# sid2364/dna-sequences-pg-extension

Measured on AMD Instinct MI355X. Metric: k-mers/sec for k=31 count over 3 Gbase synthetic; % of HBM-read roofline, higher is better.
Workload: dtype u64; 1 GPU; config 4: k=31 count over 3000000000 synthetic bases (splitmix64 seed 0xd2a0003), unordered groups (super-k-mer partitioning), single GPU; n_bases=3000000000, k=31, distinct=2999999968

## Files before the change

dna-sequences-pg-extension_amd/csrc/dnagpu_api.hip:

```cpp
#include "host_common.hpp"

using namespace dnagpu;

static thread_local char g_err[512] = "";

void dnagpu::set_err(const char *fmt, ...)
{
    va_list ap;
    va_start(ap, fmt);
    vsnprintf(g_err, sizeof g_err, fmt, ap);
    va_end(ap);
}

extern "C" const char *dnagpu_strerror(int status)
{
    switch (status) {
    case DNAGPU_OK: return "ok";
    case DNAGPU_ERR_INVALID_K: return "Invalid k value: must be between 1 and 32";
    case DNAGPU_ERR_QKMER_LEN_MISMATCH: return "Qkmer pattern and kmer lengths do not match";
    case DNAGPU_ERR_PREFIX_TOO_LONG: return "Prefix length cannot exceed kmer length";
    case DNAGPU_ERR_QKMER_INVALID: return "Invalid Qkmer sequence: must contain valid IUPAC nucleotide codes";
    case DNAGPU_ERR_BAD_ARG: return "bad argument";
    case DNAGPU_ERR_TOO_LARGE: return "too many k-mers for one call (limit 2^32 - 1)";
    case DNAGPU_ERR_NO_DEVICE: return "no usable HIP device (gfx950 required)";
// ... 133 lines not shown
#endif
    if (e != hipSuccess) {
        (void)hipGetLastError();
        hipStreamSynchronize(ctx->stream);
        for (size_t i = 0; i < ctx->pool.size();) {
            if (!ctx->pool[i].in_use) {
                hipFree(ctx->pool[i].ptr);
                ctx->pool.erase(ctx->pool.begin() + i);
            } else {
                i++;
            }
        }
        e = hipMalloc(&p, want);
    }
    if (e != hipSuccess) {
        (void)hipGetLastError();
        set_err("hipMalloc(%zu bytes) failed: %s", want, hipGetErrorString(e));
        return DNAGPU_ERR_OOM;
    }
    ctx->pool.push_back(PoolBlock{p, want, true});
    return finish(ctx->pool.back());
}

static int pool_check_guards(dnagpu_ctx *ctx)
{
    if (!(ctx->debug_flags & DNAGPU_DEBUG_GUARD_POOL))
        return DNAGPU_OK;
    unsigned char band[POOL_GUARD];
    for (const PoolBlock &b : ctx->pool) {
        if (!b.guard_at)
            continue;
        HIP_TRY(hipMemcpy(band, static_cast<const char *>(b.ptr) + b.guard_at, POOL_GUARD, hipMemcpyDeviceToHost));
        for (size_t i = 0; i < POOL_GUARD; i++)
            if (band[i] != 0xA5) {
                set_err("pool guard: a kernel wrote %zu bytes past the end of a %zu-byte work buffer (%s)", i + 1, b.guard_at,
                        b.in_use ? "in use" : "already returned");
                return DNAGPU_ERR_INTERNAL;
            }
    }
    return DNAGPU_OK;
}

void dnagpu::pool_free(dnagpu_ctx *ctx, void *p)
{
    if (!p)
        return;
    for (PoolBlock &b : ctx->pool)
        if (b.ptr == p) {
            b.in_use = false;
            return;
        }
}

HistPtr dnagpu::hist_new(u64 total, bool sorted)
{
    HistPtr h(new (std::nothrow) dnagpu_hist());
    if (h) {
        h->total = total;
        h->sorted = sorted;
    }
    return h;
}

void dnagpu::hist_adopt(PoolScope &ps, dnagpu_hist *h, u64 *keys, u32 *counts, u64 *seg_off, u32 *seg_cnt, u32 n_segs, u64 n_distinct,
                        bool sorted, u64 extent)
{
    h->keys = keys;
    h->counts = counts;
    h->seg_off = seg_off;
    h->seg_cnt = seg_cnt;
    h->n_segs = n_segs;
    h->n_distinct = n_distinct;
    h->sorted = sorted;
    h->extent = extent;
    ps.release(keys);
    ps.release(counts);
    ps.release(seg_off);
    ps.release(seg_cnt);
}

int dnagpu::hist_adopt_one_segment(dnagpu_ctx *ctx, PoolScope &ps, dnagpu_hist *h, u64 *keys, u32 *counts, u64 n_groups, bool sorted)
{
    u64 *dir = nullptr;
    RC_TRY(ps.alloc(2, &dir));
    const u32 words[3] = {0, 0, (u32)n_groups};
    HIP_TRY(poke(dir, words, sizeof words, ctx->stream));
    HIP_TRY(hipStreamSynchronize(ctx->stream));
    hist_adopt(ps, h, keys, counts, dir, reinterpret_cast<u32 *>(dir + 1), 1, n_groups, sorted, 0);
    return DNAGPU_OK;
}

extern "C" int dnagpu_init(int device, dnagpu_ctx **out_ctx)
{
    return guarded([&]() -> int {
    if (!out_ctx)
        return DNAGPU_ERR_BAD_ARG;
    *out_ctx = nullptr;
    int n = 0;
    hipError_t e = hipGetDeviceCount(&n);
    if (e != hipSuccess || n <= 0) {
        (void)hipGetLastError();
        set_err("hipGetDeviceCount: %s (%d devices)", hipGetErrorString(e), n);
        return DNAGPU_ERR_NO_DEVICE;
    }
    if (device < 0 || device >= n) {
        set_err("device %d out of range (%d devices)", device, n);
        return DNAGPU_ERR_NO_DEVICE;
    }
    HIP_TRY(hipSetDevice(device));
    dnagpu_ctx *ctx = new (std::nothrow) dnagpu_ctx();
    if (!ctx)
        return DNAGPU_ERR_OOM;
    ctx->device = device;
    ctx->profiling = false;
    ctx->last_times.n = 0;
    e = hipStreamCreateWithFlags(&ctx->stream, hipStreamNonBlocking);
    if (e != hipSuccess) {
        set_err("hipStreamCreate: %s", hipGetErrorString(e));
        delete ctx;
        return DNAGPU_ERR_HIP;
    }
    ctx->mailbox = nullptr;
    ctx->debug_flags = 0;
    e = hipHostMalloc(reinterpret_cast<void **>(&ctx->mailbox), MAILBOX_BYTES, hipHostMallocDefault);
    if (e == hipSuccess)
        memset(ctx->mailbox, 0, MAILBOX_BYTES);
    if (e != hipSuccess) {
        set_err("hipHostMalloc: %s", hipGetErrorString(e));
        hipStreamDestroy(ctx->stream);
        delete ctx;
        return DNAGPU_ERR_OOM;
    }
    *out_ctx = ctx;
    return DNAGPU_OK;
    });
}

extern "C" void dnagpu_destroy(dnagpu_ctx *ctx)
{
    if (!ctx)
        return;
    hipSetDevice(ctx->device);
    hipStreamSynchronize(ctx->stream);
    for (PoolBlock &b : ctx->pool)
        hipFree(b.ptr);
    for (hipEvent_t e : ctx->ev)
        hipEventDestroy(e);
    hipStreamDestroy(ctx->stream);
    if (ctx->mailbox)
        hipHostFree(ctx->mailbox);
    delete ctx;
}

extern "C" int dnagpu_synchronize(dnagpu_ctx *ctx)
{
    return guarded([&]() -> int {
    if (!ctx)
        return DNAGPU_ERR_BAD_ARG;
    HIP_TRY(hipStreamSynchronize(ctx->stream));
    return pool_check_guards(ctx);
    });
}

extern "C" void *dnagpu_stream(dnagpu_ctx *ctx) { return ctx ? (void *)ctx->stream : nullptr; }

extern "C" int dnagpu_trim(dnagpu_ctx *ctx)
{
    return guarded([&]() -> int {
    if (!ctx)
        return DNAGPU_ERR_BAD_ARG;
    HIP_TRY(hipStreamSynchronize(ctx->stream));
    for (size_t i = 0; i < ctx->pool.size();) {
        if (!ctx->pool[i].in_use) {
            hipFree(ctx->pool[i].ptr);
            ctx->pool.erase(ctx->pool.begin() + i);
        } else {
            i++;
        }
    }
    return DNAGPU_OK;
    });
}

extern "C" uint64_t dnagpu_device_bytes(dnagpu_ctx *ctx)
{
    uint64_t t = 0;
    if (ctx)
        for (PoolBlock &b : ctx->pool)
            t += b.size;
    return t;
}

extern "C" int dnagpu_buffer_alloc(dnagpu_ctx *ctx, uint64_t bytes, void **dev_ptr)
{
    return guarded([&]() -> int {
    if (!ctx || !dev_ptr)
        return DNAGPU_ERR_BAD_ARG;
    HIP_TRY(hipSetDevice(ctx->device));
    return pool_alloc(ctx, (size_t)bytes, dev_ptr);
    });
// ... 1075 lines not shown
```

dna-sequences-pg-extension_amd/csrc/host_common.hpp:

```cpp
#pragma once
#include <hip/hip_runtime.h>

#include <algorithm>
#include <atomic>
#include <chrono>
#include <cmath>
#include <cstdarg>
#include <cstdio>
#include <cstdlib>
#include <cstring>
#include <initializer_list>
#include <memory>
#include <new>
#include <vector>

#include "../../include/dnagpu.h"
#include "kernels.hpp"

namespace dnagpu {
void set_err(const char *fmt, ...);

#ifdef DNAGPU_STAMPS
inline const char *diag_env(const char *name) { return getenv(name); }
#else
// ... 5 lines not shown
        hipError_t e_ = (expr);                                                              \
        if (e_ != hipSuccess) {                                                              \
            set_err("%s failed: %s (%s:%d)", #expr, hipGetErrorString(e_), __FILE__, __LINE__); \
            return e_ == hipErrorOutOfMemory ? DNAGPU_ERR_OOM : DNAGPU_ERR_HIP;              \
        }                                                                                    \
    } while (0)

#define RC_TRY(expr)           \
    do {                       \
        int rc_ = (expr);      \
        if (rc_ != DNAGPU_OK)  \
            return rc_;        \
    } while (0)

template <typename F>
int guarded(F &&body) noexcept
{
    try {
        return body();
    } catch (const std::bad_alloc &) {
        set_err("host allocation failed");
        return DNAGPU_ERR_OOM;
    } catch (...) {
        set_err("unexpected C++ exception");
        return DNAGPU_ERR_INTERNAL;
    }
}

struct PoolBlock {
    void *ptr;
    size_t size;
    bool in_use;
    size_t guard_at = 0;
};
constexpr size_t POOL_GUARD = 256;

constexpr size_t MAILBOX_BYTES = (size_t)1 << 20;

}
using dnagpu::u32;
using dnagpu::u64;

struct dnagpu_ctx {
    int device;
    hipStream_t stream;
    std::vector<dnagpu::PoolBlock> pool;
    bool profiling;
    dnagpu_phase_times last_times;
    std::vector<hipEvent_t> ev;
    std::vector<const char *> ev_names;
    u64 *mailbox;
    u64 mailbox_seq = 0;
    unsigned debug_flags;
};

struct dnagpu_dna {
    u64 *words;
    u64 n_words;
    u64 n_bases;
    bool owned;
    u64 *seq_starts = nullptr;
    u32 *seq_marks = nullptr;
    u64 n_seqs = 0, n_mark_words = 0;
};

struct dnagpu_hist {
    u64 *keys = nullptr;
    u32 *counts = nullptr;
    u64 n_distinct = 0;
    u64 total = 0;
    u64 *seg_off = nullptr;
    u32 *seg_cnt = nullptr;
    u32 *seg_pre = nullptr;
    u32 n_segs = 0;
    bool sorted = true;
    u64 extent = 0;
    std::vector<dnagpu_hist *> parts;
    int k = 0;
};
using HistPtr = std::unique_ptr<dnagpu_hist>;

namespace dnagpu {
hipError_t poke(void *dst, const void *src, size_t bytes, hipStream_t st);
int read_back(dnagpu_ctx *ctx, void *host, const void *dev, size_t bytes);

int pool_alloc(dnagpu_ctx *ctx, size_t bytes, void **out);
void pool_free(dnagpu_ctx *ctx, void *p);

template <typename T>
int pool_alloc_t(dnagpu_ctx *ctx, size_t n, T **out)
{
    void *p = nullptr;
    int rc = pool_alloc(ctx, n * sizeof(T), &p);
    *out = static_cast<T *>(p);
    return rc;
}

struct PoolScope {
    dnagpu_ctx *ctx;
    std::vector<void *> ptrs;
    explicit PoolScope(dnagpu_ctx *c) : ctx(c) {}
    ~PoolScope()
    {
        for (void *p : ptrs)
            pool_free(ctx, p);
    }
    template <typename T>
    int alloc(size_t n, T **out)
    {
        int rc = pool_alloc_t(ctx, n, out);
        if (rc == DNAGPU_OK)
            ptrs.push_back(*out);
        return rc;
    }
    void release(void *p)
    {
        ptrs.erase(std::remove(ptrs.begin(), ptrs.end(), p), ptrs.end());
    }
    void free_now(void *p)
    {
        release(p);
        pool_free(ctx, p);
    }
};

HistPtr hist_new(u64 total, bool sorted = true);
void hist_adopt(PoolScope &ps, dnagpu_hist *h, u64 *keys, u32 *counts, u64 *seg_off, u32 *seg_cnt, u32 n_segs, u64 n_distinct,
                bool sorted, u64 extent);
int hist_adopt_one_segment(dnagpu_ctx *ctx, PoolScope &ps, dnagpu_hist *h, u64 *keys, u32 *counts, u64 n_groups, bool sorted);

void prof_begin(dnagpu_ctx *ctx);
void prof_mark(dnagpu_ctx *ctx, const char *name);
void prof_end(dnagpu_ctx *ctx);

inline u64 words_for(u64 n_bases) { return (n_bases + 31) / 32; }
int check_range(const dnagpu_dna *dna, int k, u64 first, u64 count);

#pragma GCC visibility push(hidden)
constexpr u64 U32_MAX64 = 0xFFFFFFFFull;

// ... 151 lines not shown
```

dna-sequences-pg-extension_amd/csrc/sk_host.hip:

```cpp
#include "host_common.hpp"

using namespace dnagpu;


constexpr u64 SK_LEAF_MEAN = 2500;
constexpr u64 SK_MID_LIMIT = (u64)1 << 27;
#ifndef SK_MID_RECORDS_LOG2
#define SK_MID_RECORDS_LOG2 16
#endif
constexpr u32 SK_MID_RECORDS = 1u << SK_MID_RECORDS_LOG2;
constexpr u64 SK_BIG_LIMIT = 0xFFFFFFFFull;
constexpr int SK_B1_MAX = 9;
constexpr u64 SK_SLAB_MIN_ROWS = (u64)1 << 29;

template <typename T>
static int alloc1(PoolScope &ps, size_t n, T **out, size_t per = 1)
{
    return ps.alloc(std::max<size_t>(n, 1) * per, out);
}

static u32 sk_chunk_len(u64 x, u64 target = 4096, u64 tile = 8192)
{
    const u64 len = std::max<u64>(4 * tile, (x + target - 1) / target);
    return (u32)((len + tile - 1) / tile * tile);
// ... 122 lines not shown
static int sk_level0(dnagpu_ctx *ctx, PoolScope &ps, SkParts &p, const SkRows &rows, bool room_for_level1)
{
    hipStream_t st = ctx->stream;
    const dnagpu_dna *dna = rows.dna;
    const int k = p.k, b1 = p.g.b1, r0bits = p.g.r0bits;
    const u32 c0n = p.g.c0n;
    Node *cur = nullptr;
    u32 chunk_rows = 0;
    SkLevel l0;
    RC_TRY(sk_level0_begin(ctx, ps, rows.n, r0bits, 4096, &cur, &chunk_rows, &l0));
    prof_mark(ctx, "sk_hist0");
    HIP_TRY(launch_sk_level0(false, l0.chunks, l0.n_chunks, dna->words, dna->n_words, rows.first, k, c0n, (u32)b1, (u32)r0bits,
                             l0.hist, nullptr, nullptr, st, nullptr, rows.marks, rows.n_mark_words));
    prof_mark(ctx, "sk_prefix0");
    HIP_TRY(launch_level_prefix(cur, l0.chunks, l0.n_chunks, 1, chunk_rows, l0.hist, l0.tot, st));
    HIP_TRY(launch_level_children(cur, 1, l0.tot, l0.next, nullptr, nullptr, nullptr, 0, st));
    std::vector<Node> kids(l0.n_next);
    RC_TRY(read_back(ctx, kids.data(), l0.next, (size_t)l0.n_next * sizeof(Node)));
    std::vector<u32> &lens = p.lens;
    lens.resize(kids.size());
    u64 n_recs = 0;
    for (size_t i = 0; i < kids.size(); i++) {
        lens[i] = kids[i].len;
        n_recs += kids[i].len;
    }
    if (n_recs > 0xFFFFFFFFull)
        return DNAGPU_ERR_TOO_LARGE;
    void *rec0 = nullptr;
    u64 cap = std::max<u64>(n_recs, 1);
    if (room_for_level1) {
        u64 span = 0;
        const bool even = sk_even(lens.data(), (u32)lens.size(), 1.02, b1, &span);
        if (span <= 0xFFFFFFFFull)
            cap = std::max(cap, span);
        if ((ctx->debug_flags & DNAGPU_DEBUG_SAMPLE1) || !even) {
            const u64 roomy = n_recs + n_recs / 3 + ((u64)lens.size() << b1) * 136;
            if (roomy <= 0xFFFFFFFFull)
                cap = std::max(cap, roomy);
        }
    }
    RC_TRY(pool_alloc(ctx, (size_t)cap * 16, &rec0));
    ps.ptrs.push_back(rec0);
    prof_mark(ctx, "sk_scatter0");
    HIP_TRY(launch_sk_level0(true, l0.chunks, l0.n_chunks, dna->words, dna->n_words, rows.first, k, c0n, (u32)b1, (u32)r0bits,
                             l0.hist, l0.tot, rec0, st, nullptr, rows.marks, rows.n_mark_words));
    p.rec0 = rec0;
    p.rec0_cap = cap;
    p.coarse = l0.next;
    p.n_coarse = l0.n_next;
    p.n_recs = n_recs;
    return DNAGPU_OK;
}

static int sk_level0_slab(dnagpu_ctx *ctx, PoolScope &ps, SkParts &p, const SkRows &rows, bool *ok)
{
    hipStream_t st = ctx->stream;
    const dnagpu_dna *dna = rows.dna;
    const SkGeom &g = p.g;
    const int k = p.k;
    const u64 first = rows.first, n = rows.n;
    *ok = false;
    const u32 r0n = 1u << g.r0bits;
    const u64 tile = (u64)sk_tile_rows();
    Node *cur = nullptr;
    u32 chunk_rows = 0;
    SkLevel l0;
    RC_TRY(sk_level0_begin(ctx, ps, n, g.r0bits, 1024, &cur, &chunk_rows, &l0));
    if (l0.n_chunks == 0)
        return DNAGPU_OK;
    const u64 samp_len = 4 * tile, samp_stride = 64 * samp_len;
    const u32 n_samp = (u32)((n + samp_stride - 1) / samp_stride);
    u64 sampled = 0;
    for (u32 i = 0; i < n_samp; i++)
        sampled += std::min<u64>(samp_len, n - (u64)i * samp_stride);
    Chunk *samp = nullptr;
    u32 *est = nullptr, *slab = nullptr;
    Node *nodes = nullptr;
    RC_TRY(ps.alloc((size_t)n_samp, &samp));
    RC_TRY(ps.alloc((size_t)sk_max_c0(), &est));
    RC_TRY(ps.alloc((size_t)sk_slab_words(), &slab));
    RC_TRY(ps.alloc((size_t)r0n, &nodes));
    prof_mark(ctx, "sk_sample0");
    HIP_TRY(hipMemsetAsync(est, 0, (size_t)sk_max_c0() * sizeof(u32), st));
    HIP_TRY(launch_sk_sample_chunks(samp, n_samp, (u32)samp_stride, (u32)samp_len, (u32)n, st));
    HIP_TRY(launch_sk_level0(false, samp, n_samp, dna->words, dna->n_words, first, k, g.c0n, (u32)g.b1, (u32)g.r0bits, nullptr, nullptr,
                             nullptr, st, est, rows.marks, rows.n_mark_words));
    HIP_TRY(launch_sk_slab_init(est, (u32)g.r0bits, chunk_rows, (u32)sampled, l0.n_chunks, slab, nodes, st));
    std::vector<u32> h_est(r0n);
    RC_TRY(read_back(ctx, h_est.data(), est, (size_t)r0n * sizeof(u32)));
    u64 tot = 0, span = 0, span1 = 0;
    p.lens.assign(r0n, 0);
    for (u32 d = 0; d < r0n; d++) {
        tot += h_est[d];
        const u64 len = (u64)sk_slab_cap(h_est[d], chunk_rows, sampled) * l0.n_chunks;
        span += len;
        if (len > 0xFFFFFFFFull)
            return DNAGPU_OK;
        p.lens[d] = (u32)len;
        span1 += sk_spec_span((u32)len, g.b1);
    }
    if (tot == 0 || !sk_even(h_est.data(), r0n, 1.05) || span > 0xFFFFFFFFull)
        return DNAGPU_OK;
    const u64 cap = std::max<u64>(span, span1 <= 0xFFFFFFFFull ? span1 : 0);
    void *rec0 = nullptr;
    RC_TRY(pool_alloc(ctx, (size_t)std::max<u64>(cap, 1) * 16, &rec0));
    prof_mark(ctx, "sk_scatter0");
    const hipError_t e = launch_sk_level0(true, l0.chunks, l0.n_chunks, dna->words, dna->n_words, first, k, g.c0n, (u32)g.b1,
                                          (u32)g.r0bits, nullptr, nullptr, rec0, st, slab, rows.marks, rows.n_mark_words);
    u32 status[2] = {1, 0};
    int rc = e == hipSuccess ? read_back(ctx, status, slab + 18 * (size_t)sk_max_c0(), sizeof status) : DNAGPU_ERR_HIP;
    if (rc != DNAGPU_OK || status[0] || status[1] != (u32)span || (ctx->debug_flags & DNAGPU_DEBUG_SLAB0_OVERFLOW)) {
        pool_free(ctx, rec0);
        if (e != hipSuccess)
            set_err("sk_scatter0 (slabs): %s", hipGetErrorString(e));
        return rc;
    }
    ps.ptrs.push_back(rec0);
    p.rec0 = rec0;
    p.rec0_cap = cap;
    p.coarse = nodes;
    p.n_coarse = r0n;
    p.n_recs = span;
    *ok = true;
    return DNAGPU_OK;
}


struct SkL1 {
    SkLevel lv;
    u32 chunk_recs = 0;
    u32 *kcount = nullptr;
    u32 *d_lens = nullptr;
    u32 *gcur = nullptr;
    std::vector<u32> kc, rcn;
    u64 span = 0;
    u32 *rstart = nullptr, *rcapv = nullptr;
    void *rec1 = nullptr;
    bool rec1_kept = false;
};

enum class SkL1Route {
    Exact,
    Speculative,
    SpeculativeSampled,
};

static int sk_l1_plan(dnagpu_ctx *ctx, PoolScope &ps, const SkParts &p, SkL1 &l1)
{
    hipStream_t st = ctx->stream;
    l1.chunk_recs = sk_chunk_len(p.n_recs);
    prof_mark(ctx, "sk_plan1");
    RC_TRY(sk_level_begin(ctx, ps, p.coarse, p.n_coarse, p.g.b1, l1.chunk_recs, &l1.lv));
    const u32 n_mid = l1.lv.n_next;
    RC_TRY(alloc1(ps, n_mid, &l1.kcount));
    HIP_TRY(hipMemsetAsync(l1.kcount, 0, (size_t)std::max<u32>(n_mid, 1) * sizeof(u32), st));
    RC_TRY(ps.alloc((size_t)n_mid + 4, &l1.d_lens));
    RC_TRY(alloc1(ps, l1.lv.n_chunks, &l1.gcur, ROW_STRIDE));
    l1.kc.resize(n_mid);
    l1.rcn.resize((size_t)n_mid + 4);
    return DNAGPU_OK;
}

static int sk_l1_lens_to_host(dnagpu_ctx *ctx, SkL1 &l1, u32 extra)
{
    hipStream_t st = ctx->stream;
    const size_t nb = (size_t)l1.lv.n_next * sizeof(u32), nb2 = nb + (size_t)extra * sizeof(u32);
    if (nb + nb2 <= MAILBOX_BYTES - 8) {
        char *mb = reinterpret_cast<char *>(ctx->mailbox);
        HIP_TRY(hipMemcpyAsync(mb, l1.kcount, nb, hipMemcpyDeviceToHost, st));
        HIP_TRY(hipMemcpyAsync(mb + nb, l1.d_lens, nb2, hipMemcpyDeviceToHost, st));
        HIP_TRY(hipStreamSynchronize(st));
        memcpy(l1.kc.data(), mb, nb);
        memcpy(l1.rcn.data(), mb + nb, nb2);
    } else {
        HIP_TRY(hipMemcpyAsync(l1.kc.data(), l1.kcount, nb, hipMemcpyDeviceToHost, st));
        RC_TRY(read_back(ctx, l1.rcn.data(), l1.d_lens, nb2));
    }
    return DNAGPU_OK;
}

static int sk_l1_route(dnagpu_ctx *ctx, PoolScope &ps, const SkParts &p, SkL1 &l1, SkL1Route *route)
{
    hipStream_t st = ctx->stream;
    const u32 n_coarse = p.n_coarse, n_mid = l1.lv.n_next;
    const u32 *host_lens = p.lens.data();
    *route = SkL1Route::Exact;
    if (p.lens.empty() || (ctx->debug_flags & DNAGPU_DEBUG_NO_SPEC1) || n_coarse > (u32)sk_max_c0() || l1.lv.n_chunks == 0)
        return DNAGPU_OK;
    u64 span = 0;
    const bool even = sk_even(host_lens, n_coarse, 1.02, p.g.b1, &span);
    const bool force_sample = (ctx->debug_flags & DNAGPU_DEBUG_SAMPLE1) != 0;
    if (even && !force_sample) {
        if (span <= p.rec0_cap && span <= 0xFFFFFFFFull) {
            l1.span = span;
            *route = SkL1Route::Speculative;
        }
        return DNAGPU_OK;
    }
    std::vector<Chunk> samp;
    const u32 slen = sk_sample1_len(), sstep = slen * sk_sample1_every();
    for (u32 i = 0; i < n_coarse; i++)
        for (u64 off = 0; off < host_lens[i]; off += sstep) {
            Chunk c;
            c.node = i;
            c.off = (u32)off;
            c.len = (u32)std::min<u64>(slen, host_lens[i] - off);
            c.pad = 0;
            samp.push_back(c);
        }
    Chunk *d_samp = nullptr;
    u32 *est = nullptr, *stmp = nullptr, *tot1 = nullptr;
    RC_TRY(alloc1(ps, samp.size(), &d_samp));
    RC_TRY(ps.alloc((size_t)n_mid, &est));
    RC_TRY(ps.alloc((size_t)n_mid, &l1.rcapv));
    RC_TRY(ps.alloc((size_t)n_mid, &l1.rstart));
    RC_TRY(ps.alloc((size_t)scan_tmp_words(n_mid), &stmp));
    RC_TRY(ps.alloc(1, &tot1));
    prof_mark(ctx, "sk_sample1");
    if (!samp.empty())
        HIP_TRY(hipMemcpyAsync(d_samp, samp.data(), samp.size() * sizeof(Chunk), hipMemcpyHostToDevice, st));
    HIP_TRY(launch_sk_sampled_regions(p.coarse, d_samp, (u32)samp.size(), p.rec0, n_mid, est, l1.rcapv, l1.rstart, stmp, tot1, st));
    u32 total = 0;
    RC_TRY(read_back(ctx, &total, tot1, sizeof total));
    u64 chk = 0;
    for (u32 i = 0; i < n_coarse; i++)
        chk += host_lens[i];
    if ((u64)total >= chk && (u64)total <= p.rec0_cap) {
        l1.span = total;
        *route = SkL1Route::SpeculativeSampled;
    }
    return DNAGPU_OK;
}

static int sk_l1_speculative(dnagpu_ctx *ctx, PoolScope &ps, const SkParts &p, SkL1 &l1, SkL1Route route, bool *moved)
{
    hipStream_t st = ctx->stream;
    const bool sampled = route == SkL1Route::SpeculativeSampled;
    const u32 n_mid = l1.lv.n_next;
    u32 *const rstart = sampled ? l1.rstart : nullptr, *const rcapv = sampled ? l1.rcapv : nullptr;
    u32 *sp = nullptr;
    RC_TRY(ps.alloc((size_t)2 * p.n_coarse, &sp));
    u32 *status = l1.d_lens + n_mid;
    prof_mark(ctx, "sk_spec1");
    HIP_TRY(launch_sk_spec_regions(p.coarse, p.n_coarse, sp, status, l1.gcur, st, rstart));
    RC_TRY(pool_alloc(ctx, (size_t)std::max<u64>(std::max(p.n_recs, l1.span), 1) * 16, &l1.rec1));
    ps.ptrs.push_back(l1.rec1);
    prof_mark(ctx, "sk_scatter1");
    HIP_TRY(launch_sk_scatter1_spec(p.coarse, l1.lv.chunks, l1.lv.n_chunks, p.rec0, l1.rec1, l1.gcur, sp, l1.kcount, status + 2, st,
                                    rstart, rcapv));
    HIP_TRY(launch_sk_spec_nodes(p.coarse, p.n_coarse, sp, l1.gcur, l1.lv.next, status + 2, st, rstart, rcapv));
    HIP_TRY(launch_sk_node_lens(l1.lv.next, n_mid, l1.d_lens, st));
    RC_TRY(sk_l1_lens_to_host(ctx, l1, 3));
    const u32 *stw = l1.rcn.data() + n_mid;
    *moved = !((!sampled && stw[0] != (u32)l1.span) || (!sampled && stw[1]) || stw[2] ||
               (ctx->debug_flags & DNAGPU_DEBUG_SPEC1_OVERFLOW));
    if (!*moved)
        HIP_TRY(hipMemsetAsync(l1.kcount, 0, (size_t)std::max<u32>(n_mid, 1) * sizeof(u32), st));
    return DNAGPU_OK;
}

static int sk_l1_histogram(dnagpu_ctx *ctx, const SkParts &p, SkL1 &l1)
{
    hipStream_t st = ctx->stream;
    const SkLevel &lv = l1.lv;
    prof_mark(ctx, "sk_hist1");
    HIP_TRY(launch_sk_hist1(p.coarse, lv.chunks, lv.n_chunks, p.rec0, lv.hist, l1.kcount, st));
    prof_mark(ctx, "sk_prefix1");
    HIP_TRY(launch_level_prefix(p.coarse, lv.chunks, lv.n_chunks, p.n_coarse, l1.chunk_recs, lv.hist, lv.tot, st, p.n_coarse));
    HIP_TRY(launch_level_children(p.coarse, p.n_coarse, lv.tot, lv.next, nullptr, nullptr, nullptr, 0, st));
    HIP_TRY(launch_sk_node_lens(lv.next, lv.n_next, l1.d_lens, st));
    return sk_l1_lens_to_host(ctx, l1, 0);
}

static int sk_l1_census(unsigned debug_flags, const SkL1 &l1, SkParts &p, std::vector<u32> *heavy_idx)
{
    const std::vector<u32> &kc = l1.kc, &rcn = l1.rcn;
    const u32 n_mid = l1.lv.n_next;
    const u64 mid_limit = p.g.mid_limit;
    const bool forced = (debug_flags & DNAGPU_DEBUG_FORCE_SUPERKMER) != 0;
    auto is_heavy = [&](u32 i) { return kc[i] > mid_limit || (!forced && rcn[i] > SK_MID_RECORDS); };
    u64 run = 0;
    bool any_heavy = false;
    for (u32 i = 0; i < n_mid; i++) {
        run += kc[i];
        any_heavy = any_heavy || is_heavy(i);
    }
    if (p.n_expected != 0 && run != p.n_expected) {
        set_err("super-k-mer partition lost rows: %llu of %llu", (unsigned long long)run, (unsigned long long)p.n_expected);
        return DNAGPU_ERR_INTERNAL;
    }
    if (run > 0xFFFFFFFFull)
        return DNAGPU_ERR_TOO_LARGE;
    p.n_kmers = run;
    if (!any_heavy)
        return DNAGPU_OK;
    for (u32 i = 0; i < n_mid; i++)
        if (is_heavy(i)) {
            heavy_idx->push_back(i);
            p.heavy.total += kc[i];
        }
    if (((debug_flags & DNAGPU_DEBUG_HEAVY_EXPAND) && p.heavy.total * 2 > run) || heavy_idx->size() > 32768)
        return DNAGPU_SK_SKEWED;
    return DNAGPU_OK;
}

static int sk_l1_scatter(dnagpu_ctx *ctx, PoolScope &ps, const SkParts &p, SkL1 &l1)
{
    hipStream_t st = ctx->stream;
    const SkLevel &lv = l1.lv;
    if (!l1.rec1) {
        RC_TRY(pool_alloc(ctx, (size_t)std::max<u64>(p.n_recs, 1) * 16, &l1.rec1));
// ... 17 lines not shown
    const u32 nh = (u32)heavy_idx.size();
    u32 *d_idx = nullptr;
    Node *hnodes = nullptr;
    RC_TRY(ps.alloc((size_t)nh, &d_idx));
    RC_TRY(ps.alloc((size_t)nh, &hnodes));
    HIP_TRY(hipMemcpyAsync(d_idx, heavy_idx.data(), (size_t)nh * sizeof(u32), hipMemcpyHostToDevice, st));
    HIP_TRY(launch_sk_take_heavy(l1.lv.next, d_idx, nh, l1.kcount, hnodes, st));
    HIP_TRY(hipStreamSynchronize(st));
    if (ctx->debug_flags & DNAGPU_DEBUG_HEAVY_EXPAND) {
        p.heavy.nodes = hnodes;
        p.heavy.n = nh;
        p.heavy.recs = l1.rec1;
        l1.rec1_kept = true;
        return DNAGPU_OK;
    }
    u64 hrecs = 0;
    for (u32 i : heavy_idx)
        hrecs += l1.rcn[i];
    const u32 chunk_h = sk_chunk_len(hrecs);
    SkLevel &lh = split->lv;
    prof_mark(ctx, "sk_heavy_split");
    RC_TRY(sk_level_begin(ctx, ps, hnodes, nh, 4, chunk_h, &lh));
    RC_TRY(alloc1(ps, lh.n_next, &split->kcount));
    HIP_TRY(hipMemsetAsync(split->kcount, 0, (size_t)std::max<u32>(lh.n_next, 1) * sizeof(u32), st));
    HIP_TRY(launch_sk_hist1(hnodes, lh.chunks, lh.n_chunks, l1.rec1, lh.hist, split->kcount, st, true));
    HIP_TRY(launch_level_prefix(hnodes, lh.chunks, lh.n_chunks, nh, chunk_h, lh.hist, lh.tot, st, nh));
    HIP_TRY(launch_level_children(hnodes, nh, lh.tot, lh.next, nullptr, nullptr, nullptr, 0, st));
    HIP_TRY(launch_sk_scatter1(hnodes, lh.chunks, lh.n_chunks, l1.rec1, p.rec0, lh.hist, lh.tot, st, true));
    p.heavy.total = 0;
    return DNAGPU_OK;
}

static int sk_level2(dnagpu_ctx *ctx, PoolScope &ps, SkParts &p, SkL1 &l1, const SkSplit &split)
{
    hipStream_t st = ctx->stream;
    const u32 n_mid = l1.lv.n_next, n_split = split.lv.n_next;
    Node *fn = nullptr;
    RC_TRY(ps.alloc((size_t)n_mid * 16 + n_split, &fn));
    prof_mark(ctx, "sk_regroup");
    bool any_long = false;
    for (u32 i = 0; i < n_mid && !any_long; i++)
        any_long = l1.rcn[i] > (u32)sk_regroup_tile();
    HIP_TRY(launch_sk_regroup(l1.lv.next, n_mid, l1.rec1, p.rec0, fn, any_long, st));
    if (n_split)
        HIP_TRY(launch_sk_heavy_finals(split.lv.next, n_split, split.kcount, fn + (size_t)n_mid * 16, st));
    if (!l1.rec1_kept)
        ps.free_now(l1.rec1);
    p.recs = p.rec0;
    p.fin = fn;
    p.n_fin = n_mid * 16 + n_split;
    return DNAGPU_OK;
}

static int sk_levels12(dnagpu_ctx *ctx, PoolScope &ps, SkParts &p)
{
    SkL1 l1;
    SkL1Route route;
    RC_TRY(sk_l1_plan(ctx, ps, p, l1));
    RC_TRY(sk_l1_route(ctx, ps, p, l1, &route));
    bool moved = false;
    if (route != SkL1Route::Exact)
        RC_TRY(sk_l1_speculative(ctx, ps, p, l1, route, &moved));
    if (!moved)
        RC_TRY(sk_l1_histogram(ctx, p, l1));
    std::vector<u32> heavy_idx;
    RC_TRY(sk_l1_census(ctx->debug_flags, l1, p, &heavy_idx));
    if (!moved)
        RC_TRY(sk_l1_scatter(ctx, ps, p, l1));
    SkSplit split;
    if (!heavy_idx.empty())
        RC_TRY(sk_heavy_take(ctx, ps, p, l1, heavy_idx, &split));
    return sk_level2(ctx, ps, p, l1, split);
}


struct SkTail {
    u32 *f_small = nullptr, *f_big = nullptr, *k_range = nullptr, *f_over = nullptr;
    u32 *scan_tmp = nullptr, *totals = nullptr;
    u32 *list_small = nullptr, *off_small = nullptr, *list_big = nullptr, *off_big = nullptr;
    u32 n_small = 0, n_big = 0, big_kmers = 0;
    u64 small_keys = 0;
    u64 out_cap = 0;
    u64 *cursor = nullptr;
    u64 *ok = nullptr;
    u32 *oc = nullptr;
    u64 *seg_off_fin = nullptr;
    u32 *seg_cnt_fin = nullptr;
    u32 *big_status = nullptr;
    Node *over_nodes = nullptr;
    u32 n_over = 0;
    u64 over_keys = 0;
    TreeResult tr = {};
    u64 *seg_off = nullptr;
    u32 *seg_cnt = nullptr;
    u32 n_segs = 0;
};

static int sk_tail_select(dnagpu_ctx *ctx, PoolScope &ps, const SkParts &p, u64 n, SkTail &t)
{
    hipStream_t st = ctx->stream;
    const u32 n_fin = p.n_fin;
    prof_mark(ctx, "sk_select");
    RC_TRY(ps.alloc((size_t)n_fin, &t.f_small));
    RC_TRY(ps.alloc((size_t)n_fin, &t.f_big));
    RC_TRY(ps.alloc((size_t)n_fin, &t.k_range));
    RC_TRY(ps.alloc((size_t)scan_tmp_words(n_fin) * 4, &t.scan_tmp));
    RC_TRY(ps.alloc(8, &t.totals));
    RC_TRY(ps.alloc((size_t)n_fin, &t.list_small));
    RC_TRY(ps.alloc((size_t)n_fin, &t.off_small));
    RC_TRY(ps.alloc((size_t)n_fin, &t.f_over));
    HIP_TRY(launch_sk_select_flags(p.fin, n_fin, (u32)sk_count_cap(), (u32)SK_BIG_LIMIT, t.f_small, t.f_big, t.k_range, t.f_over, st));
    HIP_TRY(launch_scan_u32_multi(scans_in_place({t.f_small, t.f_big, t.k_range, t.f_over}, t.totals, t.scan_tmp), 4, n_fin, st));
    u32 ht[4] = {0, 0, 0, 0};
    RC_TRY(read_back(ctx, ht, t.totals, sizeof ht));
    t.n_small = ht[0];
    t.n_big = ht[1];
    t.small_keys = ht[2];
    t.big_kmers = ht[3];
    t.out_cap = n + t.big_kmers;
    RC_TRY(alloc1(ps, t.n_big, &t.list_big));
    RC_TRY(alloc1(ps, t.n_big, &t.off_big));
    HIP_TRY(launch_sk_select_lists(p.fin, n_fin, (u32)sk_count_cap(), (u32)SK_BIG_LIMIT, t.f_small, t.f_big, t.k_range, t.list_small,
                                   t.off_small, t.list_big, t.off_big, st));
    return DNAGPU_OK;
}
// ... 152 lines not shown
        RC_TRY(read_back(ctx, &nl, left + 2 * (size_t)t.n_small, 4));
        fprintf(stderr, "[sk count] %u small buckets, %u left to sk_count by sk_count_clean\n", t.n_small, nl);
    }
#endif
    return DNAGPU_OK;
}

static int sk_tail_finish(dnagpu_ctx *ctx, PoolScope &ps, const SkTail &t, u64 n, dnagpu_hist *h)
{
    prof_mark(ctx, "end");
    u64 fin_ctr[3] = {0, 0, 0};
    RC_TRY(read_back(ctx, fin_ctr, t.cursor, 24));
    const u64 extent = fin_ctr[0];
    const u64 total_groups = fin_ctr[2] + (extent - t.small_keys);
    if (fin_ctr[1] != 0) {
        set_err("super-k-mer count: %llu buckets whose records expand to a different number of k-mers than the partition counted",
                (unsigned long long)fin_ctr[1]);
        return DNAGPU_ERR_INTERNAL;
    }
    if (extent > t.out_cap) {
        set_err("super-k-mer count: %llu output slots used, %llu allocated", (unsigned long long)extent, (unsigned long long)t.out_cap);
        return DNAGPU_ERR_INTERNAL;
    }
    if (total_groups > n) {
        set_err("super-k-mer count: %llu groups for %llu rows", (unsigned long long)total_groups, (unsigned long long)n);
        return DNAGPU_ERR_INTERNAL;
    }
    h->total = n;
    hist_adopt(ps, h, t.ok, t.oc, t.seg_off, t.seg_cnt, t.n_segs, total_groups, false, extent);
    return DNAGPU_OK;
}

static int count_sk_tail(dnagpu_ctx *ctx, PoolScope &ps, const SkParts &p, u64 n, dnagpu_hist *h)
{
    SkTail t;
    RC_TRY(sk_tail_select(ctx, ps, p, n, t));
    RC_TRY(sk_tail_outputs(ctx, ps, p, t));
    if (t.n_big)
        RC_TRY(sk_tail_count_big(ctx, ps, p, t));
    RC_TRY(sk_tail_select_over(ctx, ps, p, t));
    RC_TRY(sk_tail_tree(ctx, ps, p, t));
    RC_TRY(sk_tail_leaves(ctx, ps, p, t));
    RC_TRY(sk_tail_count(ctx, ps, p, t));
    return sk_tail_finish(ctx, ps, t, n, h);
}

int dnagpu::count_sk(dnagpu_ctx *ctx, const SkRows &rows, int k, dnagpu_hist *h, u64 n_kmers_expected)
{
    PoolScope ps(ctx);
    SkParts p;
    p.g = sk_geometry(ctx, std::max<u64>(n_kmers_expected, 1), k);
    p.k = k;
    p.n_expected = n_kmers_expected;
    bool slabs = false;
    const unsigned dbg = ctx->debug_flags;
    if (!(dbg & DNAGPU_DEBUG_NO_SLAB0) && (rows.n >= SK_SLAB_MIN_ROWS || (dbg & (DNAGPU_DEBUG_SLAB0 | DNAGPU_DEBUG_SLAB0_OVERFLOW))))
        RC_TRY(sk_level0_slab(ctx, ps, p, rows, &slabs));
    if (!slabs)
        RC_TRY(sk_level0(ctx, ps, p, rows, true));
    RC_TRY(sk_levels12(ctx, ps, p));
    return count_sk_tail(ctx, ps, p, n_kmers_expected, h);
}

u64 dnagpu::sk_received_cap(const std::vector<u64> &blen, u32 n_coarse, const SkGeom &g)
{
    u64 n_recs = 0, span = 0;
    for (u32 d = 0; d < n_coarse; d++) {
        n_recs += blen[d];
        span += sk_spec_span((u32)std::min<u64>(blen[d], 0xFFFFFFFFull), g.b1);
    }
    return span <= 0xFFFFFFFFull ? std::max(n_recs, span) : n_recs;
}

int dnagpu::count_sk_received(dnagpu_ctx *ctx, void *rec0, const std::vector<u64> &boff, const std::vector<u64> &blen, const SkGeom &g,
                              int k, dnagpu_hist *h, u64 rec0_cap)
{
    hipStream_t st = ctx->stream;
    PoolScope ps(ctx);
    ps.ptrs.push_back(rec0);
    SkParts p;
    p.g = g;
    p.k = k;
    p.rec0 = rec0;
    p.rec0_cap = rec0_cap;
    p.n_coarse = 1u << g.r0bits;
    p.n_recs = boff[p.n_coarse];
    p.lens.resize(p.n_coarse);
    std::vector<Node> hn(p.n_coarse);
    for (u32 d = 0; d < p.n_coarse; d++) {
        memset(&hn[d], 0, sizeof(Node));
        hn[d].start = (u32)boff[d];
        hn[d].len = p.lens[d] = (u32)blen[d];
        hn[d].meta = (u32)(32 - g.r0bits);
    }
    RC_TRY(ps.alloc((size_t)p.n_coarse, &p.coarse));
    HIP_TRY(hipMemcpyAsync(p.coarse, hn.data(), (size_t)p.n_coarse * sizeof(Node), hipMemcpyHostToDevice, st));
    HIP_TRY(hipStreamSynchronize(st));
    int rc = sk_levels12(ctx, ps, p);
    if (rc == DNAGPU_SK_SKEWED) {
        p.heavy = SkHeavy();
        p.heavy.nodes = p.coarse;
        p.heavy.n = p.n_coarse;
        p.heavy.recs = rec0;
        p.heavy.total = p.n_kmers;
        p.heavy.counted = false;
        p.n_fin = 0;
        rc = DNAGPU_OK;
    }
    RC_TRY(rc);
    return count_sk_tail(ctx, ps, p, p.n_kmers, h);
}

static int count_sk_records(dnagpu_ctx *ctx, const void *const *pieces, const u64 *piece_len, const u32 *piece_bucket, u32 n_pieces,
// ... 123 lines not shown
```

Before: 162.9 billion k-mers/s.

## Pipeline level-0 slab scatter with level-1 speculative scatter on a side stream

Splits the level-0 slab scatter into several pieces by chunk range and, after each piece, launches the level-1 speculative scatter for that piece's records on a second non-blocking stream, synchronised with events. This overlaps the two scatter passes instead of running them back to back, and folds the level-0 overflow status readback into the level-1 length readback, saving one host sync. It adds a side stream, per-piece node/chunk tables built on the host, and an extra readback of the coarse nodes. The path only runs for large inputs without sequence marks when the plain speculative route applies.

```diff
diff --git a/dna-sequences-pg-extension_amd/csrc/dnagpu_api.hip b/dna-sequences-pg-extension_amd/csrc/dnagpu_api.hip
--- a/dna-sequences-pg-extension_amd/csrc/dnagpu_api.hip
+++ b/dna-sequences-pg-extension_amd/csrc/dnagpu_api.hip
@@ -209,6 +209,18 @@
         }
 }
 
+int dnagpu::side_stream(dnagpu_ctx *ctx, size_t n_events)
+{
+    if (!ctx->stream2)
+        HIP_TRY(hipStreamCreateWithFlags(&ctx->stream2, hipStreamNonBlocking));
+    while (ctx->sync_ev.size() < n_events) {
+        hipEvent_t e;
+        HIP_TRY(hipEventCreateWithFlags(&e, hipEventDisableTiming));
+        ctx->sync_ev.push_back(e);
+    }
+    return DNAGPU_OK;
+}
+
 HistPtr dnagpu::hist_new(u64 total, bool sorted)
 {
     HistPtr h(new (std::nothrow) dnagpu_hist());
@@ -299,10 +311,16 @@
         return;
     hipSetDevice(ctx->device);
     hipStreamSynchronize(ctx->stream);
+    if (ctx->stream2)
+        hipStreamSynchronize(ctx->stream2);
     for (PoolBlock &b : ctx->pool)
         hipFree(b.ptr);
     for (hipEvent_t e : ctx->ev)
         hipEventDestroy(e);
+    for (hipEvent_t e : ctx->sync_ev)
+        hipEventDestroy(e);
+    if (ctx->stream2)
+        hipStreamDestroy(ctx->stream2);
     hipStreamDestroy(ctx->stream);
     if (ctx->mailbox)
         hipHostFree(ctx->mailbox);
diff --git a/dna-sequences-pg-extension_amd/csrc/host_common.hpp b/dna-sequences-pg-extension_amd/csrc/host_common.hpp
--- a/dna-sequences-pg-extension_amd/csrc/host_common.hpp
+++ b/dna-sequences-pg-extension_amd/csrc/host_common.hpp
@@ -81,6 +81,8 @@
     u64 *mailbox;
     u64 mailbox_seq = 0;
     unsigned debug_flags;
+    hipStream_t stream2 = nullptr;
+    std::vector<hipEvent_t> sync_ev;
 };
 
 struct dnagpu_dna {
@@ -115,6 +117,7 @@
 
 int pool_alloc(dnagpu_ctx *ctx, size_t bytes, void **out);
 void pool_free(dnagpu_ctx *ctx, void *p);
+int side_stream(dnagpu_ctx *ctx, size_t n_events);
 
 template <typename T>
 int pool_alloc_t(dnagpu_ctx *ctx, size_t n, T **out)
diff --git a/dna-sequences-pg-extension_amd/csrc/sk_host.hip b/dna-sequences-pg-extension_amd/csrc/sk_host.hip
--- a/dna-sequences-pg-extension_amd/csrc/sk_host.hip
+++ b/dna-sequences-pg-extension_amd/csrc/sk_host.hip
@@ -198,7 +198,29 @@
     return DNAGPU_OK;
 }
 
-static int sk_level0_slab(dnagpu_ctx *ctx, PoolScope &ps, SkParts &p, const SkRows &rows, bool *ok)
+#ifndef SK_L0_PIECES_N
+#define SK_L0_PIECES_N 4
+#endif
+constexpr u32 SK_L0_PIECES = SK_L0_PIECES_N;
+constexpr u64 SK_PIPE_MIN_ROWS = (u64)5 << 29;
+constexpr u64 SK_SLAB_CHUNKS = 1024, SK_SLAB_CHUNKS_PIPED = 512 * SK_L0_PIECES;
+
+struct SkSlab {
+    SkLevel l0;
+    u32 *slab = nullptr;
+    std::vector<u32> cap;
+    u64 span = 0;
+    bool pipe = false;
+};
+
+static void sk_piece_range(u32 n_chunks, u32 i, u32 *a, u32 *b)
+{
+    const u32 per = (n_chunks + SK_L0_PIECES - 1) / SK_L0_PIECES;
+    *a = std::min(n_chunks, i * per);
+    *b = std::min(n_chunks, (i + 1) * per);
+}
+
+static int sk_slab_begin(dnagpu_ctx *ctx, PoolScope &ps, SkParts &p, const SkRows &rows, SkSlab &sl, bool *ok)
 {
     hipStream_t st = ctx->stream;
     const dnagpu_dna *dna = rows.dna;
@@ -210,8 +232,8 @@
     const u64 tile = (u64)sk_tile_rows();
     Node *cur = nullptr;
     u32 chunk_rows = 0;
-    SkLevel l0;
-    RC_TRY(sk_level0_begin(ctx, ps, n, g.r0bits, 1024, &cur, &chunk_rows, &l0));
+    SkLevel &l0 = sl.l0;
+    RC_TRY(sk_level0_begin(ctx, ps, n, g.r0bits, sl.pipe ? SK_SLAB_CHUNKS_PIPED : SK_SLAB_CHUNKS, &cur, &chunk_rows, &l0));
     if (l0.n_chunks == 0)
         return DNAGPU_OK;
     const u64 samp_len = 4 * tile, samp_stride = 64 * samp_len;
@@ -220,29 +242,31 @@
     for (u32 i = 0; i < n_samp; i++)
         sampled += std::min<u64>(samp_len, n - (u64)i * samp_stride);
     Chunk *samp = nullptr;
-    u32 *est = nullptr, *slab = nullptr;
+    u32 *est = nullptr;
     Node *nodes = nullptr;
     RC_TRY(ps.alloc((size_t)n_samp, &samp));
     RC_TRY(ps.alloc((size_t)sk_max_c0(), &est));
-    RC_TRY(ps.alloc((size_t)sk_slab_words(), &slab));
+    RC_TRY(ps.alloc((size_t)sk_slab_words(), &sl.slab));
     RC_TRY(ps.alloc((size_t)r0n, &nodes));
     prof_mark(ctx, "sk_sample0");
     HIP_TRY(hipMemsetAsync(est, 0, (size_t)sk_max_c0() * sizeof(u32), st));
     HIP_TRY(launch_sk_sample_chunks(samp, n_samp, (u32)samp_stride, (u32)samp_len, (u32)n, st));
     HIP_TRY(launch_sk_level0(false, samp, n_samp, dna->words, dna->n_words, first, k, g.c0n, (u32)g.b1, (u32)g.r0bits, nullptr, nullptr,
                              nullptr, st, est, rows.marks, rows.n_mark_words));
-    HIP_TRY(launch_sk_slab_init(est, (u32)g.r0bits, chunk_rows, (u32)sampled, l0.n_chunks, slab, nodes, st));
+    HIP_TRY(launch_sk_slab_init(est, (u32)g.r0bits, chunk_rows, (u32)sampled, l0.n_chunks, sl.slab, nodes, st));
     std::vector<u32> h_est(r0n);
     RC_TRY(read_back(ctx, h_est.data(), est, (size_t)r0n * sizeof(u32)));
     u64 tot = 0, span = 0, span1 = 0;
-    p.lens.assign(r0n, 0);
+    std::vector<u32> lens(r0n, 0);
+    sl.cap.assign(r0n, 0);
     for (u32 d = 0; d < r0n; d++) {
         tot += h_est[d];
-        const u64 len = (u64)sk_slab_cap(h_est[d], chunk_rows, sampled) * l0.n_chunks;
+        sl.cap[d] = sk_slab_cap(h_est[d], chunk_rows, sampled);
+        const u64 len = (u64)sl.cap[d] * l0.n_chunks;
         span += len;
         if (len > 0xFFFFFFFFull)
             return DNAGPU_OK;
-        p.lens[d] = (u32)len;
+        lens[d] = (u32)len;
         span1 += sk_spec_span((u32)len, g.b1);
     }
     if (tot == 0 || !sk_even(h_est.data(), r0n, 1.05) || span > 0xFFFFFFFFull)
@@ -250,18 +274,9 @@
     const u64 cap = std::max<u64>(span, span1 <= 0xFFFFFFFFull ? span1 : 0);
     void *rec0 = nullptr;
     RC_TRY(pool_alloc(ctx, (size_t)std::max<u64>(cap, 1) * 16, &rec0));
-    prof_mark(ctx, "sk_scatter0");
-    const hipError_t e = launch_sk_level0(true, l0.chunks, l0.n_chunks, dna->words, dna->n_words, first, k, g.c0n, (u32)g.b1,
-                                          (u32)g.r0bits, nullptr, nullptr, rec0, st, slab, rows.marks, rows.n_mark_words);
-    u32 status[2] = {1, 0};
-    int rc = e == hipSuccess ? read_back(ctx, status, slab + 18 * (size_t)sk_max_c0(), sizeof status) : DNAGPU_ERR_HIP;
-    if (rc != DNAGPU_OK || status[0] || status[1] != (u32)span || (ctx->debug_flags & DNAGPU_DEBUG_SLAB0_OVERFLOW)) {
-        pool_free(ctx, rec0);
-        if (e != hipSuccess)
-            set_err("sk_scatter0 (slabs): %s", hipGetErrorString(e));
-        return rc;
-    }
     ps.ptrs.push_back(rec0);
+    sl.span = span;
+    p.lens.swap(lens);
     p.rec0 = rec0;
     p.rec0_cap = cap;
     p.coarse = nodes;
@@ -269,6 +284,34 @@
     p.n_recs = span;
     *ok = true;
     return DNAGPU_OK;
+}
+
+static int sk_slab_piece(dnagpu_ctx *ctx, const SkParts &p, const SkRows &rows, const SkSlab &sl, u32 a, u32 b)
+{
+    const dnagpu_dna *dna = rows.dna;
+    const SkGeom &g = p.g;
+    const hipError_t e = launch_sk_level0(true, sl.l0.chunks + a, b - a, dna->words, dna->n_words, rows.first, p.k, g.c0n, (u32)g.b1,
+                                          (u32)g.r0bits, nullptr, nullptr, p.rec0, ctx->stream, sl.slab, rows.marks, rows.n_mark_words);
+    if (e != hipSuccess) {
+        set_err("sk_scatter0 (slabs): %s", hipGetErrorString(e));
+        return DNAGPU_ERR_HIP;
+    }
+    return DNAGPU_OK;
+}
+
+static bool sk_slab_ok(const dnagpu_ctx *ctx, const SkSlab &sl, const u32 status[2])
+{
+    return !status[0] && status[1] == (u32)sl.span && !(ctx->debug_flags & DNAGPU_DEBUG_SLAB0_OVERFLOW);
+}
+
+static void sk_slab_give_up(PoolScope &ps, SkParts &p)
+{
+    ps.free_now(p.rec0);
+    p.rec0 = nullptr;
+    p.rec0_cap = p.n_recs = 0;
+    p.coarse = nullptr;
+    p.n_coarse = 0;
+    p.lens.clear();
 }
 
 
@@ -281,6 +324,7 @@
     std::vector<u32> kc, rcn;
     u64 span = 0;
     u32 *rstart = nullptr, *rcapv = nullptr;
+    u32 *sp = nullptr;
     void *rec1 = nullptr;
     bool rec1_kept = false;
 };
@@ -307,22 +351,45 @@
     return DNAGPU_OK;
 }
 
-static int sk_l1_lens_to_host(dnagpu_ctx *ctx, SkL1 &l1, u32 extra)
-{
-    hipStream_t st = ctx->stream;
-    const size_t nb = (size_t)l1.lv.n_next * sizeof(u32), nb2 = nb + (size_t)extra * sizeof(u32);
-    if (nb + nb2 <= MAILBOX_BYTES - 8) {
+static int sk_l1_lens_to_host(dnagpu_ctx *ctx, SkL1 &l1, u32 extra, const u32 *more = nullptr, u32 *more_host = nullptr)
+{
+    hipStream_t st = ctx->stream;
+    const size_t nb = (size_t)l1.lv.n_next * sizeof(u32), nb2 = nb + (size_t)extra * sizeof(u32), nb3 = more ? 2 * sizeof(u32) : 0;
+    if (nb + nb2 + nb3 <= MAILBOX_BYTES - 8) {
         char *mb = reinterpret_cast<char *>(ctx->mailbox);
         HIP_TRY(hipMemcpyAsync(mb, l1.kcount, nb, hipMemcpyDeviceToHost, st));
         HIP_TRY(hipMemcpyAsync(mb + nb, l1.d_lens, nb2, hipMemcpyDeviceToHost, st));
+        if (more)
+            HIP_TRY(hipMemcpyAsync(mb + nb + nb2, more, nb3, hipMemcpyDeviceToHost, st));
         HIP_TRY(hipStreamSynchronize(st));
         memcpy(l1.kc.data(), mb, nb);
         memcpy(l1.rcn.data(), mb + nb, nb2);
+        if (more)
+            memcpy(more_host, mb + nb + nb2, nb3);
     } else {
         HIP_TRY(hipMemcpyAsync(l1.kc.data(), l1.kcount, nb, hipMemcpyDeviceToHost, st));
         RC_TRY(read_back(ctx, l1.rcn.data(), l1.d_lens, nb2));
-    }
-    return DNAGPU_OK;
+        if (more)
+            RC_TRY(read_back(ctx, more_host, more, nb3));
+    }
+    return DNAGPU_OK;
+}
+
+static void sk_l1_route_plain(const dnagpu_ctx *ctx, const SkParts &p, SkL1 &l1, bool *any_spec, bool *plain)
+{
+    *any_spec = *plain = false;
+    if (p.lens.empty() || (ctx->debug_flags & DNAGPU_DEBUG_NO_SPEC1) || p.n_coarse > (u32)sk_max_c0() || l1.lv.n_chunks == 0)
+        return;
+    u64 span = 0;
+    const bool even = sk_even(p.lens.data(), p.n_coarse, 1.02, p.g.b1, &span);
+    if (even && !(ctx->debug_flags & DNAGPU_DEBUG_SAMPLE1)) {
+        if (span <= p.rec0_cap && span <= 0xFFFFFFFFull) {
+            l1.span = span;
+            *any_spec = *plain = true;
+        }
+        return;
+    }
+    *any_spec = true;
 }
 
 static int sk_l1_route(dnagpu_ctx *ctx, PoolScope &ps, const SkParts &p, SkL1 &l1, SkL1Route *route)
@@ -331,18 +398,12 @@
     const u32 n_coarse = p.n_coarse, n_mid = l1.lv.n_next;
     const u32 *host_lens = p.lens.data();
     *route = SkL1Route::Exact;
-    if (p.lens.empty() || (ctx->debug_flags & DNAGPU_DEBUG_NO_SPEC1) || n_coarse > (u32)sk_max_c0() || l1.lv.n_chunks == 0)
+    bool any_spec = false, plain = false;
+    sk_l1_route_plain(ctx, p, l1, &any_spec, &plain);
+    if (plain)
+        *route = SkL1Route::Speculative;
+    if (!any_spec || plain)
         return DNAGPU_OK;
-    u64 span = 0;
-    const bool even = sk_even(host_lens, n_coarse, 1.02, p.g.b1, &span);
-    const bool force_sample = (ctx->debug_flags & DNAGPU_DEBUG_SAMPLE1) != 0;
-    if (even && !force_sample) {
-        if (span <= p.rec0_cap && span <= 0xFFFFFFFFull) {
-            l1.span = span;
-            *route = SkL1Route::Speculative;
-        }
-        return DNAGPU_OK;
-    }
     std::vector<Chunk> samp;
     const u32 slen = sk_sample1_len(), sstep = slen * sk_sample1_every();
     for (u32 i = 0; i < n_coarse; i++)
@@ -378,31 +439,46 @@
     return DNAGPU_OK;
 }
 
-static int sk_l1_speculative(dnagpu_ctx *ctx, PoolScope &ps, const SkParts &p, SkL1 &l1, SkL1Route route, bool *moved)
+static int sk_l1_spec_begin(dnagpu_ctx *ctx, PoolScope &ps, const SkParts &p, SkL1 &l1, SkL1Route route)
+{
+    const bool sampled = route == SkL1Route::SpeculativeSampled;
+    RC_TRY(ps.alloc((size_t)2 * p.n_coarse, &l1.sp));
+    u32 *status = l1.d_lens + l1.lv.n_next;
+    prof_mark(ctx, "sk_spec1");
+    HIP_TRY(launch_sk_spec_regions(p.coarse, p.n_coarse, l1.sp, status, l1.gcur, ctx->stream, sampled ? l1.rstart : nullptr));
+    RC_TRY(pool_alloc(ctx, (size_t)std::max<u64>(std::max(p.n_recs, l1.span), 1) * 16, &l1.rec1));
+    ps.ptrs.push_back(l1.rec1);
+    return DNAGPU_OK;
+}
+
+static int sk_l1_spec_end(dnagpu_ctx *ctx, const SkParts &p, SkL1 &l1, SkL1Route route, bool *moved, const u32 *l0_status = nullptr,
+                          u32 *l0_status_host = nullptr)
 {
     hipStream_t st = ctx->stream;
     const bool sampled = route == SkL1Route::SpeculativeSampled;
     const u32 n_mid = l1.lv.n_next;
     u32 *const rstart = sampled ? l1.rstart : nullptr, *const rcapv = sampled ? l1.rcapv : nullptr;
-    u32 *sp = nullptr;
-    RC_TRY(ps.alloc((size_t)2 * p.n_coarse, &sp));
     u32 *status = l1.d_lens + n_mid;
-    prof_mark(ctx, "sk_spec1");
-    HIP_TRY(launch_sk_spec_regions(p.coarse, p.n_coarse, sp, status, l1.gcur, st, rstart));
-    RC_TRY(pool_alloc(ctx, (size_t)std::max<u64>(std::max(p.n_recs, l1.span), 1) * 16, &l1.rec1));
-    ps.ptrs.push_back(l1.rec1);
-    prof_mark(ctx, "sk_scatter1");
-    HIP_TRY(launch_sk_scatter1_spec(p.coarse, l1.lv.chunks, l1.lv.n_chunks, p.rec0, l1.rec1, l1.gcur, sp, l1.kcount, status + 2, st,
-                                    rstart, rcapv));
-    HIP_TRY(launch_sk_spec_nodes(p.coarse, p.n_coarse, sp, l1.gcur, l1.lv.next, status + 2, st, rstart, rcapv));
+    HIP_TRY(launch_sk_spec_nodes(p.coarse, p.n_coarse, l1.sp, l1.gcur, l1.lv.next, status + 2, st, rstart, rcapv));
     HIP_TRY(launch_sk_node_lens(l1.lv.next, n_mid, l1.d_lens, st));
-    RC_TRY(sk_l1_lens_to_host(ctx, l1, 3));
+    RC_TRY(sk_l1_lens_to_host(ctx, l1, 3, l0_status, l0_status_host));
     const u32 *stw = l1.rcn.data() + n_mid;
     *moved = !((!sampled && stw[0] != (u32)l1.span) || (!sampled && stw[1]) || stw[2] ||
                (ctx->debug_flags & DNAGPU_DEBUG_SPEC1_OVERFLOW));
     if (!*moved)
         HIP_TRY(hipMemsetAsync(l1.kcount, 0, (size_t)std::max<u32>(n_mid, 1) * sizeof(u32), st));
     return DNAGPU_OK;
+}
+
+static int sk_l1_speculative(dnagpu_ctx *ctx, PoolScope &ps, const SkParts &p, SkL1 &l1, SkL1Route route, bool *moved)
+{
+    const bool sampled = route == SkL1Route::SpeculativeSampled;
+    RC_TRY(sk_l1_spec_begin(ctx, ps, p, l1, route));
+    prof_mark(ctx, "sk_scatter1");
+    HIP_TRY(launch_sk_scatter1_spec(p.coarse, l1.lv.chunks, l1.lv.n_chunks, p.rec0, l1.rec1, l1.gcur, l1.sp, l1.kcount,
+                                    l1.d_lens + l1.lv.n_next + 2, ctx->stream, sampled ? l1.rstart : nullptr,
+                                    sampled ? l1.rcapv : nullptr));
+    return sk_l1_spec_end(ctx, p, l1, route, moved);
 }
 
 static int sk_l1_histogram(dnagpu_ctx *ctx, const SkParts &p, SkL1 &l1)
@@ -526,15 +602,8 @@
     return DNAGPU_OK;
 }
 
-static int sk_levels12(dnagpu_ctx *ctx, PoolScope &ps, SkParts &p)
-{
-    SkL1 l1;
-    SkL1Route route;
-    RC_TRY(sk_l1_plan(ctx, ps, p, l1));
-    RC_TRY(sk_l1_route(ctx, ps, p, l1, &route));
-    bool moved = false;
-    if (route != SkL1Route::Exact)
-        RC_TRY(sk_l1_speculative(ctx, ps, p, l1, route, &moved));
+static int sk_levels12_rest(dnagpu_ctx *ctx, PoolScope &ps, SkParts &p, SkL1 &l1, bool moved)
+{
     if (!moved)
         RC_TRY(sk_l1_histogram(ctx, p, l1));
     std::vector<u32> heavy_idx;
@@ -545,6 +614,133 @@
     if (!heavy_idx.empty())
         RC_TRY(sk_heavy_take(ctx, ps, p, l1, heavy_idx, &split));
     return sk_level2(ctx, ps, p, l1, split);
+}
+
+static int sk_levels12_planned(dnagpu_ctx *ctx, PoolScope &ps, SkParts &p, SkL1 &l1)
+{
+    SkL1Route route;
+    RC_TRY(sk_l1_route(ctx, ps, p, l1, &route));
+    bool moved = false;
+    if (route != SkL1Route::Exact)
+        RC_TRY(sk_l1_speculative(ctx, ps, p, l1, route, &moved));
+    return sk_levels12_rest(ctx, ps, p, l1, moved);
+}
+
+static int sk_levels12(dnagpu_ctx *ctx, PoolScope &ps, SkParts &p)
+{
+    SkL1 l1;
+    RC_TRY(sk_l1_plan(ctx, ps, p, l1));
+    return sk_levels12_planned(ctx, ps, p, l1);
+}
+
+
+struct SideWork {
+    hipStream_t s, main;
+    bool joined = false;
+    SideWork(hipStream_t side, hipStream_t main_stream) : s(side), main(main_stream) {}
+    ~SideWork()
+    {
+        if (!joined) {
+            (void)hipStreamSynchronize(s);
+            (void)hipStreamSynchronize(main);
+        }
+    }
+};
+
+static int sk_l01_piped(dnagpu_ctx *ctx, PoolScope &ps, SkParts &p, const SkRows &rows, const SkSlab &sl, SkL1 &l1, bool *slab_ok,
+                        bool *moved)
+{
+    hipStream_t st = ctx->stream;
+    const u32 n_coarse = p.n_coarse, chunk_recs = l1.chunk_recs;
+    RC_TRY(side_stream(ctx, SK_L0_PIECES + 1));
+    RC_TRY(sk_l1_spec_begin(ctx, ps, p, l1, SkL1Route::Speculative));
+    std::vector<Node> planned(n_coarse), pn;
+    RC_TRY(read_back(ctx, planned.data(), p.coarse, (size_t)n_coarse * sizeof(Node)));
+    std::vector<Chunk> pc;
+    u32 first_chunk[SK_L0_PIECES + 1];
+    for (u32 i = 0; i < SK_L0_PIECES; i++) {
+        u32 a = 0, b = 0;
+        sk_piece_range(sl.l0.n_chunks, i, &a, &b);
+        first_chunk[i] = (u32)pc.size();
+        for (u32 d = 0; d < n_coarse; d++) {
+            Node nd = planned[d];
+            nd.start += sl.cap[d] * a;
+            nd.len = sl.cap[d] * (b - a);
+            pn.push_back(nd);
+            for (u32 off = 0; nd.split && off < nd.len; off += chunk_recs) {
+                Chunk c;
+                c.node = d;
+                c.off = off;
+                c.len = std::min(chunk_recs, nd.len - off);
+                c.pad = 0;
+                pc.push_back(c);
+            }
+        }
+    }
+    first_chunk[SK_L0_PIECES] = (u32)pc.size();
+    Node *d_pn = nullptr;
+    Chunk *d_pc = nullptr;
+    RC_TRY(alloc1(ps, pn.size(), &d_pn));
+    RC_TRY(alloc1(ps, pc.size(), &d_pc));
+    SideWork side(ctx->stream2, st);
+    HIP_TRY(hipMemcpyAsync(d_pn, pn.data(), pn.size() * sizeof(Node), hipMemcpyHostToDevice, st));
+    if (!pc.empty())
+        HIP_TRY(hipMemcpyAsync(d_pc, pc.data(), pc.size() * sizeof(Chunk), hipMemcpyHostToDevice, st));
+    u32 *status1 = l1.d_lens + l1.lv.n_next;
+    prof_mark(ctx, "sk_scatter0");
+    for (u32 i = 0; i < SK_L0_PIECES; i++) {
+        u32 a = 0, b = 0;
+        sk_piece_range(sl.l0.n_chunks, i, &a, &b);
+        RC_TRY(sk_slab_piece(ctx, p, rows, sl, a, b));
+        HIP_TRY(hipEventRecord(ctx->sync_ev[i], st));
+        HIP_TRY(hipStreamWaitEvent(side.s, ctx->sync_ev[i], 0));
+        HIP_TRY(launch_sk_scatter1_spec(d_pn + (size_t)i * n_coarse, d_pc + first_chunk[i], first_chunk[i + 1] - first_chunk[i], p.rec0,
+                                        l1.rec1, l1.gcur, l1.sp, l1.kcount, status1 + 2, side.s, nullptr, nullptr));
+    }
+    prof_mark(ctx, "sk_scatter1");
+    HIP_TRY(hipEventRecord(ctx->sync_ev[SK_L0_PIECES], side.s));
+    HIP_TRY(hipStreamWaitEvent(st, ctx->sync_ev[SK_L0_PIECES], 0));
+    side.joined = true;
+    u32 status0[2] = {1, 0};
+    RC_TRY(sk_l1_spec_end(ctx, p, l1, SkL1Route::Speculative, moved, sl.slab + 18 * (size_t)sk_max_c0(), status0));
+    *slab_ok = sk_slab_ok(ctx, sl, status0);
+    if (!*slab_ok) {
+        ps.free_now(l1.rec1);
+        l1.rec1 = nullptr;
+        *moved = false;
+    }
+    return DNAGPU_OK;
+}
+
+static int sk_levels012_slab(dnagpu_ctx *ctx, PoolScope &ps, SkParts &p, const SkRows &rows, bool *done)
+{
+    *done = false;
+    SkSlab sl;
+    sl.pipe = (ctx->debug_flags & (DNAGPU_DEBUG_SLAB0 | DNAGPU_DEBUG_SLAB0_OVERFLOW)) || (!rows.marks && rows.n >= SK_PIPE_MIN_ROWS);
+    bool ok = false;
+    RC_TRY(sk_slab_begin(ctx, ps, p, rows, sl, &ok));
+    if (!ok)
+        return DNAGPU_OK;
+    SkL1 l1;
+    RC_TRY(sk_l1_plan(ctx, ps, p, l1));
+    bool any_spec = false, plain = false, moved = false;
+    sk_l1_route_plain(ctx, p, l1, &any_spec, &plain);
+    const bool piped = sl.pipe && plain;
+    if (piped) {
+        RC_TRY(sk_l01_piped(ctx, ps, p, rows, sl, l1, &ok, &moved));
+    } else {
+        prof_mark(ctx, "sk_scatter0");
+        RC_TRY(sk_slab_piece(ctx, p, rows, sl, 0, sl.l0.n_chunks));
+        u32 status0[2] = {1, 0};
+        RC_TRY(read_back(ctx, status0, sl.slab + 18 * (size_t)sk_max_c0(), sizeof status0));
+        ok = sk_slab_ok(ctx, sl, status0);
+    }
+    if (!ok) {
+        sk_slab_give_up(ps, p);
+        return DNAGPU_OK;
+    }
+    *done = true;
+    return piped ? sk_levels12_rest(ctx, ps, p, l1, moved) : sk_levels12_planned(ctx, ps, p, l1);
 }
 
 
@@ -803,13 +999,14 @@
     p.g = sk_geometry(ctx, std::max<u64>(n_kmers_expected, 1), k);
     p.k = k;
     p.n_expected = n_kmers_expected;
-    bool slabs = false;
+    bool done = false;
     const unsigned dbg = ctx->debug_flags;
     if (!(dbg & DNAGPU_DEBUG_NO_SLAB0) && (rows.n >= SK_SLAB_MIN_ROWS || (dbg & (DNAGPU_DEBUG_SLAB0 | DNAGPU_DEBUG_SLAB0_OVERFLOW))))
-        RC_TRY(sk_level0_slab(ctx, ps, p, rows, &slabs));
-    if (!slabs)
+        RC_TRY(sk_levels012_slab(ctx, ps, p, rows, &done));
+    if (!done) {
         RC_TRY(sk_level0(ctx, ps, p, rows, true));
-    RC_TRY(sk_levels12(ctx, ps, p));
+        RC_TRY(sk_levels12(ctx, ps, p));
+    }
     return count_sk_tail(ctx, ps, p, n_kmers_expected, h);
 }
 
```

Result: faster. 167.6 billion k-mers/s, median of 6 (+2.9%).
